# Mesoptier/ray-marching

Hardware: AMD Instinct MI355X
Metric: Mpixels/s at 1920x1080, 256-step march, 32-node SDF (higher is better)
Workload: dtype f32; 1 GPU; 1920x1080, g32 (31 commands / 111 words), 256 max steps, 16 rays/px, RGBA32F out; camera=still, kernel=0, specialized_kernel=True, jit_from_disk_cache=True, frames_in_flight=4

## Files before the change

ray-marching_amd/csrc/rm_abi.hip:

```cpp
#include <hip/hip_runtime.h>

#include <algorithm>
#include <cassert>
#include <cstdarg>
#include <cstdio>
#include <cstdlib>
#include <cmath>
#include <cstring>
#include <mutex>
#include <string>
#include <type_traits>
#include <vector>

#include "rm_abi.h"
#include "rm_abi_layout.h"
#include "rm_lds_layout.h"
#include "rm_decode.h"
#include "rm_jit.h"
#include "rm_device.h"
#include "rm_kernels.h"
#include "rm_interp.h"
#include "rm_kernel_v5.h"
#include "rm_query.h"
#include "rm_trace.h"
// ... 107 lines not shown
    DevBuf<char> d_swork, d_slayers, d_spoints, d_scontours, d_sattr;
    bool slice_valid = false;
    uint64_t slice_p = 0, slice_c = 0;
    uint32_t slice_layers = 0, slice_flags = 0;
    DevBuf<char> d_out;
    DevBuf<rm_uniforms> d_frames;
    int kernel = RM_KERNEL_DEFAULT;
    uint32_t refill_min_v5 = 0;
    bool cull = true;
    int balance = 3;
    int waves_per_tile = 0;
    bool wave_stats = false;
    DevBuf<unsigned long long> d_stats;
    size_t stats_valid_bytes = 0;
    DevBuf<uint32_t> d_cost, d_order;
    DevBuf<uint32_t> d_counters;
    DevBuf<uint32_t> d_measured;
    uint64_t measured_shape = 0;
    bool timing = false;
    double last_kernel_ms = 0.0;
    int specialize = 1;
    int out_format = RM_FORMAT_RGBA32F;
    int prune = 2;
    uint64_t prog_gen = 0;
    std::shared_ptr<rmjit::Entry> spec;
    uint64_t spec_gen = ~0ull;
    int spec_wpt = 0;
    int spec_pruned = 0;
    bool spec_stats = false;
    bool last_specialized = false;
// ... 198 lines not shown
    const RmDecoded& d = c->decoded;
    const V5Plan plan = plan_v5(c, L, lds);
    const bool units = plan.units;
    const int loop = plan.loop;
    c->last_loop = loop;
    const uint32_t n_tiles = ((L.W + 7u) / 8u) * ((L.rows + 7u) / 8u);
    hipFunction_t spec_fn = lds ? specialised_kernel(c, WPT) : nullptr;
    if (spec_fn) { L.spill_depth = 0u; L.n_tree = 0u; }
    if (L.n_mrec != 0u && !(spec_fn && c->spec && c->spec->material_walk))
        L.spill_depth = std::max(L.spill_depth, 2u * d.mat_spill_depth + 3u * d.mat_xform_depth);
    L.wave_dwords = rml::V5_WAVE_DWORDS - ((spec_fn && c->spec && c->spec->taps4 && L.n_mrec == 0u) ? rml::V5_TN_DWORDS : 0u);
    const size_t shmem = rml::MarchLds(WPT, L.wave_dwords, L.spill_depth, L.n_cone, L.n_slab, lds, L.n_rec, L.n_grp, L.n_tree, L.n_mrec != 0u).bytes;
    if (shmem > rml::kLdsLaunchLimit) return fail(c, RM_ERR_TOO_LARGE, "program needs %zu bytes of LDS per tile", shmem);
    if (int rc = c->d_cost.reserve(c, (size_t)n_tiles * n_frames)) return rc;
    if (int rc = c->d_order.reserve(c, (size_t)n_tiles * n_frames)) return rc;
    if (int rc = c->d_counters.reserve(c, (size_t)n_frames * 4u)) return rc;
    hipLaunchKernelGGL(rmk::rm_tile_pre_v5, dim3((n_tiles + rmk::V5_PRE_BLOCK - 1u) / rmk::V5_PRE_BLOCK, 1, n_frames),
                       dim3(64u * rmk::V5_PRE_TILES), rml::CullLds(L.n_cone, L.n_slab, true).bytes, s, L, c->d_cost.p, n_tiles);
    const uint32_t* prev = nullptr;
    uint32_t* measured = nullptr;
    if (c->balance == 3) {
        const size_t need = (size_t)n_tiles * n_frames;
        if (need > c->d_measured.cap) {
            if (int rc = c->d_measured.reserve(c, need)) return rc;
            c->measured_shape = 0;
        }
        const uint64_t shape = ((uint64_t)L.W << 40) ^ ((uint64_t)L.rows << 20) ^ ((uint64_t)L.strip_rows << 12) ^
                               ((uint64_t)L.strip_first << 6) ^ (uint64_t)L.strip_stride ^ ((uint64_t)n_frames << 52) ^ 1ull;
        if (c->measured_shape == shape) prev = c->d_measured.p;
        else HIP_TRY(c, hipMemsetAsync(c->d_measured.p, 0, need * sizeof(uint32_t), s));
        c->measured_shape = shape;
        measured = c->d_measured.p;
    }
    hipLaunchKernelGGL(rmk::rm_tile_sort_v5, dim3(n_frames), dim3(1024), 0, s, L, c->d_cost.p, c->d_order.p, c->d_counters.p,
                       n_tiles, (uint32_t)c->balance, prev);
    rmk::V5Work work{c->d_order.p, c->d_counters.p, measured};
    uint32_t per_cu = (uint32_t)std::min<size_t>(32u / WPT, (160u * 1024u) / shmem);
    if (per_cu < 1u) per_cu = 1u;
    if (per_cu > 24u / WPT) per_cu = 24u / WPT;
    const uint32_t n_wg = std::min<uint32_t>(n_tiles, (uint32_t)std::max(1, c->cu_count) * per_cu);
    dim3 grid(n_wg, 1, n_frames);
    if (int rc = ensure_stats(c, L, (size_t)n_wg * n_frames * WPT)) return rc;
    if (int rc = time_begin(c, s)) return rc;
    const bool ext = d.has_extensions || !d.is_tree;
    c->last_specialized = spec_fn != nullptr;
    const bool pruning = spec_fn ? (c->spec && c->spec_pruned != rmjit::PRUNE_NONE) : units && lds;
    const uint32_t refill_auto = c->refill_min_v5 != 0u ? c->refill_min_v5 : (pruning ? 64u : 1u);
    if (spec_fn) {
        uint32_t n_tiles_arg = n_tiles, refill = refill_auto;
        void* args[] = {&L, &work, &n_tiles_arg, &refill};
        hipError_t e = hipModuleLaunchKernel(spec_fn, grid.x, grid.y, grid.z, 64u * WPT, 1, 1, (unsigned)shmem, s, args, nullptr);
// ... 1994 lines not shown
```

ray-marching_amd/csrc/rm_kernel_v5.h:

```cpp
#pragma once
#include "rm_interp.h"
#include "rm_lds_layout.h"

namespace rmk {

typedef const __attribute__((address_space(3))) float* LdsF;
RM_DEV LdsF lds_vector_base(const void* generic_lds_ptr) {
    const uint32_t s = (uint32_t)(__SIZE_TYPE__)(const __attribute__((address_space(3))) void*)generic_lds_ptr;
    uint32_t v;
    asm("v_mov_b32 %0, %1" : "=v"(v) : "s"(s));
    return (LdsF)(__SIZE_TYPE__)v;
}
template <bool FAST>
RM_DEV float map_scene_spec(LdsF lp, float qx, float qy, float qz, unsigned long long need, unsigned long long live, SqrtGuard& tiny, uint32_t& n_eval);
#ifdef RM_JIT_MATERIAL_WALK
template <bool FAST>
RM_DEV uint32_t map_scene_material_spec(const RmRecord* __restrict__ mp, float qx, float qy, float qz, SqrtGuard& tiny);
#endif
#ifdef RM_JIT_TAPS4
template <bool FAST>
RM_DEV void map_scene_taps(LdsF lp, float cx, float cy, float cz, unsigned long long need, unsigned long long live, SqrtGuard& tiny, float (&f)[4]);
#endif

constexpr float kPruneAbs = 4.0e-6f;
// ... 330 lines not shown
        finite = finite && hx < inf && hy < inf && hz < inf;
        const float M = cull_margin(cx, cy, cz, hx + hy + hz, ro, min_dist, slack);
        slab[3u * slot] = make_float4((cx - hx - M) - ro.x, (cy - hy - M) - ro.y, (cz - hz - M) - ro.z, 0.0f);
        slab[3u * slot + 1u] = make_float4((cx + hx + M) - ro.x, (cy + hy + M) - ro.y, (cz + hz + M) - ro.z, 0.0f);
        const float Rk = __builtin_sqrtf((hx + M) * (hx + M) + (hy + M) * (hy + M) + (hz + M) * (hz + M)) * (1.0f + 1.0e-5f);
        const float mx = cx - ro.x, my = cy - ro.y, mz = cz - ro.z;
        const float mm = mx * mx + my * my + mz * mz;
        const float lim = mm * (1.0f - 4.0e-6f) - Rk * Rk * (1.0f + 4.0e-6f);
        float sv = -inf;
        if (lim > 0.0f && lim < inf) sv = __builtin_sqrtf(lim) * (1.0f - 1.0e-5f) - 1.0e-5f * __builtin_sqrtf(mm);
        slab[3u * slot + 2u] = make_float4(mx, my, mz, sv);
    }
    if (!finite || !(slack < inf)) atomicOr(veto, 1u);
}

RM_DEV bool ray_misses_scene_v5(const CullTables& T, float dx, float dy, float dz) {
    bool clear = *T.veto == 0u;
    unit_dir(dx, dy, dz);
    for (uint32_t k = 0; k < T.n_cone; k++) {
        const float4 a = T.cone[k];
        const float t = __builtin_fmaf(a.z, dz, __builtin_fmaf(a.y, dy, __builtin_fmaf(a.x, dx, -a.w)));
        clear = clear && (t < 0.0f);
        if ((k & 3u) == 3u && __ballot(clear) == 0ull) return false;
    }
    if (T.n_slab == 0u || __ballot(clear) == 0ull) return clear;
    const float tiny = 1.0e-30f;
    const float ix = __builtin_amdgcn_rcpf(__builtin_copysignf(fmax_(__builtin_fabsf(dx), tiny), dx));
    const float iy = __builtin_amdgcn_rcpf(__builtin_copysignf(fmax_(__builtin_fabsf(dy), tiny), dy));
    const float iz = __builtin_amdgcn_rcpf(__builtin_copysignf(fmax_(__builtin_fabsf(dz), tiny), dz));
    for (uint32_t k = 0; k < T.n_slab; k++) {
        const float4 c = T.slab[3u * k + 2u];
        const float t = __builtin_fmaf(c.z, dz, __builtin_fmaf(c.y, dy, __builtin_fmaf(c.x, dx, -c.w)));
        if (__ballot(clear && !(t < 0.0f)) == 0ull) continue;
        const float4 a = T.slab[3u * k], b = T.slab[3u * k + 1u];
        const float x1 = a.x * ix, x2 = b.x * ix, y1 = a.y * iy, y2 = b.y * iy, z1 = a.z * iz, z2 = b.z * iz;
        const float tn = fmax_(fmin_(x1, x2), fmax_(fmin_(y1, y2), fmin_(z1, z2)));
        const float tf = fmin_(fmax_(x1, x2), fmin_(fmax_(y1, y2), fmax_(z1, z2)));
        clear = clear && !(tf >= fmax_(tn, 0.0f));
        if (__ballot(clear) == 0ull) return false;
    }
    return clear;
}

template <bool CONE, class LoadRecord>
RM_DEV float ray_bound_v5(const LoadRecord& load, uint32_t n_rec, const V4& ro, float dx, float dy, float dz, float scale, float rho = 0.0f) {
    if (!CONE) unit_dir(dx, dy, dz);
    const float tiny = 1.0e-18f;
    const float ax = fmax_(__builtin_fabsf(dx), tiny), ay = fmax_(__builtin_fabsf(dy), tiny), az = fmax_(__builtin_fabsf(dz), tiny);
    const float ix = __builtin_amdgcn_rcpf(__builtin_copysignf(ax, dx)), iy = __builtin_amdgcn_rcpf(__builtin_copysignf(ay, dy));
    const float iz = __builtin_amdgcn_rcpf(__builtin_copysignf(az, dz));
    const float wxy = (ax * ay) * __builtin_amdgcn_rcpf(ax + ay), wxz = (ax * az) * __builtin_amdgcn_rcpf(ax + az);
    const float wyz = (ay * az) * __builtin_amdgcn_rcpf(ay + az);
    const float lower = 2.0e-6f * scale;
    const float inf = __uint_as_float(0x7F800000u);
    float acc = inf, spilled = inf;
// ... 63 lines not shown
    }
    return acc;
}
template <bool CONE, class LoadRecord>
RM_DEV bool ray_misses_by_bounds_v5(const LoadRecord& load, uint32_t n_rec, const V4& ro, float dx, float dy, float dz, float min_dist,
                                    float scale, float rho = 0.0f) {
    const float acc = ray_bound_v5<CONE>(load, n_rec, ro, dx, dy, dz, scale, rho);
    const float margin = fmax_(min_dist, 0.0f) * 1.01f + 1.0e-4f * scale;
    return acc > margin;
}

struct V5Work {
    const uint32_t* order;
    uint32_t* counters;
    uint32_t* measured;
};

RM_DEV float select_by_mask(float a, float b, unsigned long long m) {
    float r;
    asm("v_cndmask_b32_e64 %0, %1, %2, %3" : "=v"(r) : "v"(a), "v"(b), "s"(m));
    return r;
}
RM_DEV uint32_t select_by_mask(uint32_t a, uint32_t b, unsigned long long m) {
    uint32_t r;
    asm("v_cndmask_b32_e64 %0, %1, %2, %3" : "=v"(r) : "v"(a), "v"(b), "s"(m));
    return r;
}
RM_DEV bool lane_of(unsigned long long m, uint32_t lane) {
    uint32_t r;
    asm("v_cndmask_b32_e64 %0, 0, 1, %1" : "=v"(r) : "s"(m));
// ... 18 lines not shown
    float* sq_v = reinterpret_cast<float*>(wbase + WL::sq_v / 4u);
    uint32_t* hq_rid = wbase + WL::hq_rid / 4u;
    float* hq_v = reinterpret_cast<float*>(wbase + WL::hq_v / 4u);
    float* wxy = reinterpret_cast<float*>(wbase + WL::wxy / 4u);
    float* tn = reinterpret_cast<float*>(wbase + WL::tn / 4u);
    uint32_t* after = smem + V5_POOL + WPT * L.wave_dwords;
    float* spill = reinterpret_cast<float*>(after) + wave * (L.spill_depth * 64u) + lane;
    float4* t_cone = reinterpret_cast<float4*>(after + WPT * L.spill_depth * 64u);
    float4* t_slab = t_cone + L.n_cone;
    uint32_t* lprog = reinterpret_cast<uint32_t*>(t_slab + 3u * L.n_slab);
    uint32_t* s_next = lprog + (PROG_IN_LDS ? (L.n_rec + L.n_grp + L.n_tree) * 8u : 0u);
    uint32_t* s_tile = s_next + 1;
    uint32_t* s_veto = s_next + 2;
    float* s_off = reinterpret_cast<float*>(s_next + rml::kMarchCtlBytes / 4u);
    uint8_t* rmat = reinterpret_cast<uint8_t*>(s_next) + rml::kMarchCtlBytes + rml::kMarchOffBytes;
    const bool tagged = MAT && L.n_mrec != 0u;
    constexpr uint32_t TAP_IDLE = MAT ? 5u : 4u;
    const CullTables cullt{t_cone, t_slab, s_veto, L.n_cone, L.n_slab};

    rm_uniforms u = L.u;
    if (L.frames) u = L.frames[blockIdx.z];
    const uint32_t tiles_x = (L.W + 7u) / 8u;
    const uint32_t* order = work.order + (size_t)blockIdx.z * n_tiles;
    uint32_t* counters = work.counters + 4u * blockIdx.z;
    const uint32_t n_active = counters[0];

    const V4 ro = matvec(u.inv_view, 0.0f, 0.0f, 0.0f, 1.0f);
    const float prune_scale = L.scene_scale + ((__builtin_fabsf(ro.x) + __builtin_fabsf(ro.y)) + __builtin_fabsf(ro.z));
    const float eps = 0.0001f;
    if (PROG_IN_LDS) {
// ... 110 lines not shown
        s_next[3] = 0u;
    }
    __syncthreads();
    const uint32_t slot = *s_tile;
    if (slot >= n_active) break;
    const uint32_t tile = order[slot];
    const uint32_t tile_x = tile % tiles_x, tile_y = tile / tiles_x;
    n_tiles_done++;
    const unsigned long long tile_t0 = work.measured ? __builtin_amdgcn_s_memrealtime() : 0ull;

    if (lane < 16u) {
        const uint32_t k = lane & 7u, tx = tile_x * 8u + k, ty = tile_y * 8u + k;
        wxy[lane] = lane < 8u ? screen_x(tx < L.W ? tx : L.W - 1u, L.W)
                              : screen_y(rm_global_row(L, ty < L.rows ? ty : L.rows - 1u), L.H);
    }
    __builtin_amdgcn_fence(__ATOMIC_ACQ_REL, "wavefront");

    float dx = 0.f, dy = 0.f, dz = 0.f, sc = 0.f;
    constexpr uint32_t ITR_EMPTY = 0x80000000u, ITR_RETIRED = 0x40000000u;
    uint32_t itr = ITR_EMPTY;
    auto lane_empty = [&]() { return (int32_t)itr < 0; };
    auto lane_marching = [&]() { return itr < ITR_RETIRED; };
    const uint32_t iter_limit = L.max_iter << 10;
    float thr_base = inf_f;
    uint32_t rq_pos = 0u, rq_cnt = 0u, sq_n = 0u, hq_n = 0u;
    uint32_t tap_t = TAP_IDLE, tap_n = 0u;
    bool pool_open = true;

    auto flush_misses = [&]() {
        __builtin_amdgcn_fence(__ATOMIC_ACQ_REL, "wavefront");
// ... 16 lines not shown
                        }
                        uint32_t base = 0u;
                        if (lane == 0u) base = atomicAdd(s_next, 64u);
                        base = __builtin_amdgcn_readfirstlane(base);
                        if (base >= V5_POOL) { pool_open = false; continue; }
                        n_prod++;
                        const uint32_t blk = (uint32_t)(0xEDB87421A965FC30ull >> (4u * (base >> 6))) & 15u;
                        uint32_t ln = lane;
                        asm volatile("" : "+v"(ln));
                        const uint32_t bpx = 2u * (blk & 3u) + (ln & 1u), bpy = 2u * (blk >> 2) + ((ln >> 1) & 1u), s = ln >> 2;
                        const uint32_t r = s * 64u + bpy * 8u + bpx;
                        float gx, gy, gz;
                        gen_ray_at<true>(u.inv_proj, u.inv_view, ro, wxy[bpx], wxy[8u + bpy], s_off[2u * s], s_off[2u * s + 1u], gx, gy, gz);
                        const bool finite_d = __builtin_fabsf(gx) < inf_f && __builtin_fabsf(gy) < inf_f && __builtin_fabsf(gz) < inf_f;
                        const bool test_rays = (L.flags & 1u) != 0u && __builtin_amdgcn_readfirstlane(s_next[3]) < 4u;
                        bool culled = L.max_iter == 0u || (start == START_DONE && finite_d) || (test_rays && ray_misses_scene_v5(cullt, gx, gy, gz));
#if !defined(RM_JIT_TU) || defined(RM_JIT_BOUND_WALK)
                        if (test_rays && (L.flags & 32u) && (*s_veto & 1u) == 0u && bound_scale < 1.0e12f && __ballot(!culled) != 0ull)
                            culled = culled || ray_misses_by_bounds_v5<false>(load_record, L.n_rec, ro, gx, gy, gz, L.min_dist, bound_scale);
#endif
                        if (test_rays && base < 256u && __ballot(culled) == 0ull && lane == 0u) atomicAdd(&s_next[3], 1u);
                        if (culled) res[r] = miss_code(ro, gx, gy, gz);
                        const unsigned long long keep = __ballot(!culled);
                        if (!culled) {
                            const uint32_t e = lane_rank(keep);
                            rq_rid[e] = r;
                            rq_d[e] = gx; rq_d[V5_RQ + e] = gy; rq_d[2u * V5_RQ + e] = gz;
                        }
                        rq_pos = 0u;
                        rq_cnt = (uint32_t)__popcll(keep);
                        __builtin_amdgcn_fence(__ATOMIC_ACQ_REL, "wavefront");
// ... 269 lines not shown
    cone_out[0] = cx; cone_out[1] = cy; cone_out[2] = cz;
    cone_out[3] = cone_ok ? rho : __uint_as_float(0x7FC00000u);
    return cone_ok;
}
RM_DEV float cone_noise_v5(const rm_uniforms& u, const V4& ro, uint32_t W, uint32_t H) {
    const float bx = (1.0f + 16.0f / (float)W) + 0.75f / __builtin_fabsf(u.viewport_extent[0]);
    const float by = (1.0f + 16.0f / (float)H) + 0.75f / __builtin_fabsf(u.viewport_extent[1]);
    float mag = (__builtin_fabsf(ro.x) + __builtin_fabsf(ro.y)) + __builtin_fabsf(ro.z);
#pragma unroll
    for (int k = 0; k < 4; k++)
        mag += ((__builtin_fabsf(u.inv_view[4 * k]) + __builtin_fabsf(u.inv_view[1 + 4 * k])) + __builtin_fabsf(u.inv_view[2 + 4 * k])) *
               (((__builtin_fabsf(u.inv_proj[k]) * bx + __builtin_fabsf(u.inv_proj[k + 4]) * by) + __builtin_fabsf(u.inv_proj[k + 8])) +
                __builtin_fabsf(u.inv_proj[k + 12]));
    return 1.0e-6f * mag;
}
RM_DEV bool cone_misses_tables_v5(const CullTables& T, const float2* aux, const float (&cone)[4], bool cone_ok) {
    const float cx = cone[0], cy = cone[1], cz = cone[2], rho = cone[3];
    bool clear = cone_ok && *T.veto == 0u;
    for (uint32_t k = 0; k < T.n_cone; k++) {
        const float4 a = T.cone[k];
        const float t = __builtin_fmaf(aux[k].x, rho, __builtin_fmaf(a.z, cz, __builtin_fmaf(a.y, cy, a.x * cx)));
        clear = clear && (t < a.w);
        if ((k & 3u) == 3u && __ballot(clear) == 0ull) return false;
    }
    if (T.n_slab == 0u || __ballot(clear) == 0ull) return clear;
    const float tiny = 1.0e-30f;
    const float ix = __builtin_amdgcn_rcpf(__builtin_copysignf(fmax_(__builtin_fabsf(cx), tiny), cx));
    const float iy = __builtin_amdgcn_rcpf(__builtin_copysignf(fmax_(__builtin_fabsf(cy), tiny), cy));
    const float iz = __builtin_amdgcn_rcpf(__builtin_copysignf(fmax_(__builtin_fabsf(cz), tiny), cz));
    for (uint32_t k = 0; k < T.n_slab; k++) {
        const float4 c = T.slab[3u * k + 2u];
        const float2 x = aux[T.n_cone + k];
        const float t = __builtin_fmaf(x.x, rho, __builtin_fmaf(c.z, cz, __builtin_fmaf(c.y, cy, c.x * cx)));
        if (__ballot(clear && !(t < c.w)) == 0ull) continue;
        const float infl = x.y * rho;
        const float4 a = T.slab[3u * k], b = T.slab[3u * k + 1u];
        const float x1 = (a.x - infl) * ix, x2 = (b.x + infl) * ix, y1 = (a.y - infl) * iy, y2 = (b.y + infl) * iy;
        const float z1 = (a.z - infl) * iz, z2 = (b.z + infl) * iz;
        const float tn = fmax_(fmin_(x1, x2), fmax_(fmin_(y1, y2), fmin_(z1, z2)));
        const float tf = fmin_(fmax_(x1, x2), fmin_(fmax_(y1, y2), fmax_(z1, z2)));
        clear = clear && infl < __uint_as_float(0x7F800000u) && !(tf >= fmax_(tn, 0.0f));
        if (__ballot(clear) == 0ull) return false;
    }
    return clear;
}
RM_DEV bool pixel_misses_scene_v5(const CullTables& T, const float2* aux, const float* m_proj, const float* m_view, const float* off,
                                  const V4& ro, float sx, float sy, float noise, float (&cone_out)[4], float (&corner)[4][3]) {
    const float px[2] = {sx, sx}, py[2] = {sy, sy}, ox[2] = {off[0], off[24]}, oy[2] = {off[1], off[7]};
    const bool cone_ok = rect_cone_v5(m_proj, m_view, ro, px, py, ox, oy, noise, cone_out, corner);
    return cone_misses_tables_v5(T, aux, cone_out, cone_ok);
}

RM_DEV void pixel_aux_build_v5(const float4* t_cone, const float4* t_slab, uint32_t n_cone, uint32_t n_slab, float2* t_aux, uint32_t tid,
                               uint32_t n_threads) {
    const float up = 1.0f + 1.0e-6f;
    for (uint32_t k = tid; k < n_cone + n_slab; k += n_threads) {
        float4 m;
        float radius = 0.0f;
        if (k < n_cone) {
            m = t_cone[k];
        } else {
            const uint32_t j = k - n_cone;
            m = t_slab[3u * j + 2u];
            const float4 a = t_slab[3u * j], b = t_slab[3u * j + 1u];
            const float hx = b.x - a.x, hy = b.y - a.y, hz = b.z - a.z;
// ... 50 lines not shown
        gz_lo = fmin_(gz_lo, gz); gz_hi = fmax_(gz_hi, gz);
        uniform = uniform && gx == gx && gz == gz;
    }
    const float dx_lo = Cf * gx_hi, dx_hi = Cf * gx_lo, dz_lo = Cf * gz_hi, dz_hi = Cf * gz_lo;
    const float dev_x = fmax_(__builtin_fabsf(dx_lo), __builtin_fabsf(dx_hi)), dev_z = fmax_(__builtin_fabsf(dz_lo), __builtin_fabsf(dz_hi));
    const float del_x = 4.0f * (absC * inv_my) * (Ex + ((ax_hi + Ex) * inv_my) * Ey) + 2.0e-5f * ((1.0f + __builtin_fabsf(ro.x)) + dev_x);
    const float del_z = 4.0f * (absC * inv_my) * (Ez + ((az_hi + Ez) * inv_my) * Ey) + 2.0e-5f * ((1.0f + __builtin_fabsf(ro.z)) + dev_z);
    const float nx = __builtin_rintf(((ro.x + dx_lo) - del_x) + 0.5f), nz = __builtin_rintf(((ro.z + dz_lo) - del_z) + 0.5f);
    uniform = uniform && nx == __builtin_rintf(((ro.x + dx_hi) + del_x) + 0.5f) && nz == __builtin_rintf(((ro.z + dz_hi) + del_z) + 0.5f);
    code = (__float2int_rz(nx) ^ __float2int_rz(nz)) & 1;
    return uniform;
}

constexpr uint32_t V5_TILE_CLEAR = 1u, V5_TILE_SKY = 2u, V5_TILE_CELL = 4u, V5_TILE_CODE = 8u;
RM_DEV uint32_t tile_verdict_v5(const RmLaunch& L, const rm_uniforms& u, const V4& ro, const CullTables& T, const float2* aux, const float* off,
                                bool tables, bool all_miss, uint32_t tile_x, uint32_t tile_y, float (&cone)[4]) {
    const uint32_t row = rm_global_row(L, tile_y * 8u);
    const float px[2] = {screen_x(tile_x * 8u, L.W), screen_x(tile_x * 8u + 7u, L.W)};
    const float py[2] = {screen_y(row, L.H), screen_y(row + 7u, L.H)};
    const float ox[2] = {fmin_(off[0], off[24]), fmax_(off[0], off[24])}, oy[2] = {fmax_(off[1], off[7]), fmin_(off[1], off[7])};
    float corner[4][3];
    const bool cone_ok = rect_cone_v5(u.inv_proj, u.inv_view, ro, px, py, ox, oy, cone_noise_v5(u, ro, L.W, L.H), cone, corner);
    bool clear = cone_ok && all_miss;
    if (!all_miss && tables) clear = cone_misses_tables_v5(T, aux, cone, cone_ok);
    float bx = 0.0f, by = 0.0f;
#pragma unroll
    for (int a = 0; a < 2; a++) {
        bx = fmax_(bx, __builtin_fabsf(px[a] + ox[a]));
        by = fmax_(by, __builtin_fabsf(py[a] + oy[a]));
    }
    float mag;
    int code = 0;
    const bool sky = rect_sky_v5(u, ro, corner, bx, by, mag);
    const bool cell = !sky && rect_cell_v5(u, ro, corner, bx, by, mag, code);
    bool spread = false;
#pragma unroll
    for (uint32_t c = 1; c < 4u; c++) spread = spread || corner[c][0] != corner[0][0] || corner[c][1] != corner[0][1] || corner[c][2] != corner[0][2];
    if (!spread) return 0u;
    return (clear ? V5_TILE_CLEAR : 0u) | (sky ? V5_TILE_SKY : 0u) | (cell ? V5_TILE_CELL | (code ? V5_TILE_CODE : 0u) : 0u);
}

RM_DEV CullTables stage_cull_tables(const RmLaunch& L, const V4& ro, uint32_t* smem, const rm_uniforms* u, float* off, const float2** aux,
                                    uint32_t tid, uint32_t n_threads) {
    const rml::CullLds lds(L.n_cone, L.n_slab, aux != nullptr);
    uint32_t* s_veto = lds_at<uint32_t>(smem, lds.veto);
    float4* t_cone = lds_at<float4>(smem, lds.cone);
    float4* t_slab = lds_at<float4>(smem, lds.slab);
    const bool tables = (L.flags & 1u) != 0u;
    if (tid == 0u) *s_veto = 0u;
    if (off && tid < 16u) sample_offset(*u, tid >> 2, tid & 3u, off[2u * tid], off[2u * tid + 1u]);
    __syncthreads();
    if (tables)
        for (uint32_t k = tid; k < L.n_rec; k += n_threads) cull_build_v5(L.prog[k], ro, L.min_dist, L.smooth_slack, t_cone, t_slab, s_veto, L.bounds);
    __syncthreads();
    if (aux) {
        float2* t_aux = lds_at<float2>(smem, lds.aux);
        if (tables) pixel_aux_build_v5(t_cone, t_slab, L.n_cone, L.n_slab, t_aux, tid, n_threads);
        __syncthreads();
        *aux = t_aux;
    }
    return CullTables{t_cone, t_slab, s_veto, L.n_cone, L.n_slab};
}

__global__ __launch_bounds__(64 * V5_PRE_TILES) void rm_tile_pre_v5(RmLaunch L, uint32_t* cost, uint32_t n_tiles) {
    extern __shared__ __attribute__((aligned(16))) uint32_t smem[];
    const uint32_t tid = threadIdx.x, lane = tid & 63u, wave = tid >> 6;
    rm_uniforms u = L.u;
    if (L.frames) u = L.frames[blockIdx.z];
    const V4 ro = matvec(u.inv_view, 0.0f, 0.0f, 0.0f, 1.0f);
    const bool tables = (L.flags & 1u) != 0u;
    __shared__ float s_off[32];
    __shared__ float s_sxy[V5_PRE_TILES][128];
    __shared__ uint8_t s_code[V5_PRE_TILES][64 * 16];
    __shared__ uint8_t s_list[V5_PRE_TILES][64];
    __shared__ uint8_t s_verdict[V5_PRE_BLOCK];
    __shared__ uint32_t s_claim;
    if (tid == 0u) s_claim = 0u;
    const float2* t_aux;
    const CullTables cullt = stage_cull_tables(L, ro, smem, &u, s_off, &t_aux, tid, 64u * V5_PRE_TILES);
    const uint32_t* s_veto = cullt.veto;
    const uint32_t tiles_x = (L.W + 7u) / 8u;
    const float cone_noise = cone_noise_v5(u, ro, L.W, L.H);
  auto do_tile = [&](uint32_t tile) {
    const uint32_t tile_x = tile % tiles_x, tile_y = tile / tiles_x;
    const uint32_t tx = tile_x * 8u + (lane & 7u), ty = tile_y * 8u + (lane >> 3);
    const uint32_t px = tx < L.W ? tx : L.W - 1u, ry = ty < L.rows ? ty : L.rows - 1u;
    const float sx = screen_x(px, L.W), sy = screen_y(rm_global_row(L, ry), L.H);
    float mp[16], mv[16];
#pragma unroll
    for (int k = 0; k < 16; k++) {
        mp[k] = u.inv_proj[k]; mv[k] = u.inv_view[k];
        asm volatile("" : "+v"(mp[k]), "+v"(mv[k]));
    }
    bool clear;
    float corner[4][3];
    if (L.max_iter == 0u || !tables) {
        clear = L.max_iter == 0u;
#pragma unroll
        for (uint32_t c = 0; c < 4u; c++) {
            const uint32_t s = ((c & 1u) * 3u) * 4u + (c >> 1) * 3u;
            gen_ray_unnormalized_at(mp, mv, ro, sx, sy, s_off[2u * s], s_off[2u * s + 1u], corner[c][0], corner[c][1], corner[c][2]);
        }
    } else {
        float cone[4];
        clear = pixel_misses_scene_v5(cullt, t_aux, mp, mv, s_off, ro, sx, sy, cone_noise, cone, corner);
        const float bound_scale = bound_scale_prepass_v5(L, ro);
        if ((L.flags & 32u) && (*s_veto & 1u) == 0u && bound_scale < 1.0e12f && __ballot(!clear && cone[3] == cone[3]) != 0ull) {
            const ProgSmem prog{L.prog};
            auto load_record = [&](uint32_t i, uint32_t& op, float (&p)[7]) { prog.load(i, op, p); };
            const bool by_bounds = ray_misses_by_bounds_v5<true>(load_record, L.n_rec, ro, cone[0], cone[1], cone[2], L.min_dist, bound_scale, cone[3]);
            clear = clear || (cone[3] == cone[3] && by_bounds);
        }
    }
    const uint32_t pending = (uint32_t)__popcll(__ballot(!clear));
    if (lane == 0u) cost[(size_t)blockIdx.z * n_tiles + tile] = pending;
    if (pending != 0u) return;
    const float bx = __builtin_fabsf(sx) + __builtin_fabsf(s_off[0]), by = __builtin_fabsf(sy) + __builtin_fabsf(s_off[1]);
    float mag;
    const bool sky = rect_sky_v5(u, ro, corner, bx, by, mag);
    if (__ballot(!sky) == 0ull) {
// ... 48 lines not shown
            gen_ray_at<true>(mp, mv, ro, sx, sy, s_off[2u * s], s_off[2u * s + 1u], dx, dy, dz);
            const int c = shade_floor(ro.y, ro.x, ro.z, dx, dy, dz);
            float rg, b;
            gamma_of(c, rg, b);
            tr += rg;
            tg += rg;
            tb += b;
        }
    }
    if (tx < L.W && ty < L.rows) {
        store_pixel(L, blockIdx.z, (size_t)ty * L.W + tx, tr / 16.0f, tg / 16.0f, tb / 16.0f);
    }
  };
    const uint32_t first_tile = blockIdx.x * V5_PRE_BLOCK;
    if (tid < V5_PRE_BLOCK) {
        uint32_t v = 0u;
        if ((tables || L.max_iter == 0u) && L.strip_rows % 8u == 0u) {
            const uint32_t tile = first_tile + tid < n_tiles ? first_tile + tid : n_tiles - 1u;
            float cone[4];
            v = tile_verdict_v5(L, u, ro, cullt, t_aux, s_off, tables, L.max_iter == 0u, tile % tiles_x, tile / tiles_x, cone);
            if (!(v & V5_TILE_CLEAR) || !(v & (V5_TILE_SKY | V5_TILE_CELL))) v = 0u;
        }
        s_verdict[tid] = (uint8_t)v;
    }
    __syncthreads();
    for (;;) {
        uint32_t t = 0u;
        if (lane == 0u) t = atomicAdd(&s_claim, 1u);
        t = (uint32_t)__builtin_amdgcn_readfirstlane((int)t);
        if (t >= V5_PRE_BLOCK || first_tile + t >= n_tiles) break;
        const uint32_t tile = first_tile + t, v = s_verdict[t];
        if (v == 0u) {
            do_tile(tile);
            __builtin_amdgcn_fence(__ATOMIC_ACQ_REL, "wavefront");
            continue;
        }
        float tr = 0.0f, tb = 0.0f;
        if (v & V5_TILE_CELL) {
            const float g = 0.2f * (float)((v & V5_TILE_CODE) ? 1 : 0);
            const float rg = __builtin_sqrtf(0.1f + g), b = __builtin_sqrtf(0.2f + g);
            for (uint32_t s = 0; s < 16u; s++) {
                tr += rg;
                tb += b;
            }
        }
        const uint32_t tx = (tile % tiles_x) * 8u + (lane & 7u), ty = (tile / tiles_x) * 8u + (lane >> 3);
        if (lane == 0u) cost[(size_t)blockIdx.z * n_tiles + tile] = 0u;
        if (tx < L.W && ty < L.rows) store_pixel(L, blockIdx.z, (size_t)ty * L.W + tx, tr / 16.0f, tr / 16.0f, tb / 16.0f);
// ... 89 lines not shown
        }
    }
}
#endif

#if !defined(RM_JIT_TU)
__global__ __launch_bounds__(64) void rm_selftest_cull_rays_kernel(RmLaunch L, V4 ro, const float* dirs, uint32_t n, uint32_t* out_flags,
                                                                   float* out_bound) {
    extern __shared__ __attribute__((aligned(16))) uint32_t smem[];
    const uint32_t tid = threadIdx.x;
    const bool tables = (L.flags & 1u) != 0u;
    const CullTables cullt = stage_cull_tables(L, ro, smem, nullptr, nullptr, nullptr, tid, 64u);
    const uint32_t i = blockIdx.x * 64u + tid, j = i < n ? i : n - 1u;
    const float gx = dirs[3u * j], gy = dirs[3u * j + 1u], gz = dirs[3u * j + 2u];
    const uint32_t veto = *cullt.veto;
    const bool clear = tables && ray_misses_scene_v5(cullt, gx, gy, gz);
    const float bound_scale = bound_scale_march_v5(L, ro);
    const bool walk = tables && (L.flags & 32u) && (veto & 1u) == 0u && bound_scale < 1.0e12f;
    float acc = __uint_as_float(0x7FC00000u);
    bool by_bounds = false;
    if (walk) {
        const ProgSmem prog{L.prog};
        auto load_record = [&](uint32_t r, uint32_t& op, float (&p)[7]) { prog.load(r, op, p); };
        acc = ray_bound_v5<false>(load_record, L.n_rec, ro, gx, gy, gz, bound_scale);
        by_bounds = ray_misses_by_bounds_v5<false>(load_record, L.n_rec, ro, gx, gy, gz, L.min_dist, bound_scale);
    }
    if (i < n) {
        out_flags[i] = (clear ? 1u : 0u) | ((tables && veto == 0u) ? 2u : 0u) | (walk ? 4u : 0u) | (by_bounds ? 8u : 0u) | (veto << 8);
        out_bound[i] = acc;
    }
}
// ... 4 lines not shown
    const rm_uniforms u = L.u;
    const V4 ro = matvec(u.inv_view, 0.0f, 0.0f, 0.0f, 1.0f);
    const bool tables = (L.flags & 1u) != 0u;
    const float2* t_aux;
    const CullTables cullt = stage_cull_tables(L, ro, smem, &u, s_off, &t_aux, tid, 64u);
    const uint32_t i = blockIdx.x * 64u + tid, j = i < n ? i : n - 1u;
    const float sx = screen_x(xy[2u * j], L.W), sy = screen_y(rm_global_row(L, xy[2u * j + 1u]), L.H);
    float mp[16], mv[16];
#pragma unroll
    for (int k = 0; k < 16; k++) { mp[k] = u.inv_proj[k]; mv[k] = u.inv_view[k]; }
    const float nan = __uint_as_float(0x7FC00000u), cone_noise = cone_noise_v5(u, ro, L.W, L.H);
    float cone[4] = {nan, nan, nan, nan}, corner[4][3], acc = nan;
    bool clear = false, walk = false, by_bounds = false;
    const uint32_t veto = *cullt.veto;
    if (tables) {
        clear = pixel_misses_scene_v5(cullt, t_aux, mp, mv, s_off, ro, sx, sy, cone_noise, cone, corner);
        const float bound_scale = bound_scale_prepass_v5(L, ro);
        walk = (L.flags & 32u) && (veto & 1u) == 0u && bound_scale < 1.0e12f && cone[3] == cone[3];
        if (__ballot(walk) != 0ull) {
            const ProgSmem prog{L.prog};
            auto load_record = [&](uint32_t r, uint32_t& op, float (&p)[7]) { prog.load(r, op, p); };
            const float b = ray_bound_v5<true>(load_record, L.n_rec, ro, cone[0], cone[1], cone[2], bound_scale, cone[3]);
            const bool v = ray_misses_by_bounds_v5<true>(load_record, L.n_rec, ro, cone[0], cone[1], cone[2], L.min_dist, bound_scale, cone[3]);
            if (walk) { acc = b; by_bounds = v; }
        }
    }
    if (i < n) {
        float* o = out + 8u * (size_t)i;
        o[0] = cone[0]; o[1] = cone[1]; o[2] = cone[2]; o[3] = cone[3]; o[4] = acc;
        o[5] = __uint_as_float((clear ? 1u : 0u) | ((tables && veto == 0u) ? 2u : 0u) | (walk ? 4u : 0u) | (by_bounds ? 8u : 0u));
        o[6] = 0.0f; o[7] = 0.0f;
    }
}
__global__ __launch_bounds__(64) void rm_selftest_cull_tiles_kernel(RmLaunch L, const uint32_t* xy, uint32_t n, float* out) {
    extern __shared__ __attribute__((aligned(16))) uint32_t smem[];
    __shared__ float s_off[32];
    const uint32_t tid = threadIdx.x;
    const rm_uniforms u = L.u;
    const V4 ro = matvec(u.inv_view, 0.0f, 0.0f, 0.0f, 1.0f);
    const bool tables = (L.flags & 1u) != 0u;
    const float2* t_aux;
    const CullTables cullt = stage_cull_tables(L, ro, smem, &u, s_off, &t_aux, tid, 64u);
    const uint32_t i = blockIdx.x * 64u + tid, j = i < n ? i : n - 1u;
    float cone[4];
    const uint32_t v = tile_verdict_v5(L, u, ro, cullt, t_aux, s_off, tables, L.max_iter == 0u, xy[2u * j], xy[2u * j + 1u], cone);
    if (i < n) {
        float* o = out + 8u * (size_t)i;
        o[0] = cone[0]; o[1] = cone[1]; o[2] = cone[2]; o[3] = cone[3];
        o[4] = (v & V5_TILE_CODE) ? 1.0f : 0.0f;
        o[5] = __uint_as_float(((v & V5_TILE_CLEAR) ? 1u : 0u) | ((v & V5_TILE_SKY) ? 2u : 0u) | ((v & V5_TILE_CELL) ? 4u : 0u) |
                               ((tables && *cullt.veto == 0u) ? 8u : 0u));
        o[6] = 0.0f; o[7] = 0.0f;
    }
}
__global__ __launch_bounds__(64) void rm_selftest_cull_waves_kernel(RmLaunch L, V4 ro, const float* pos, const float* thr, const unsigned long long* live,
                                                                    float extra_margin, unsigned long long* out) {
    extern __shared__ __attribute__((aligned(16))) uint32_t smem[];
    const uint32_t lane = threadIdx.x, w = blockIdx.x;
    stage_units(smem, L.prog + L.n_rec, L.n_grp, lane, 64u);
    __syncthreads();
    const float x = pos[(3u * w) * 64u + lane], y = pos[(3u * w + 1u) * 64u + lane], z = pos[(3u * w + 2u) * 64u + lane];
    const unsigned long long live_mask = live[w];
    const bool is_live = ((live_mask >> lane) & 1ull) != 0ull;
    const float prune_scale = prune_scale_v5(L, ro);
    unsigned long long need;
    if (L.unit_mode == RM_UNITS_LATTICE) need = wave_cull_lattice(smem, L.n_grp, x, y, z, thr[64u * w + lane], is_live, live_mask);
    else need = wave_cull_blend(smem, L.n_grp, L.unit_kmax, x, y, z, extra_margin, prune_scale, is_live, live_mask);
// ... 6 lines not shown
```

Before: 6706 Mpixels/s.

## Record per-tile cull-table touch masks and test only touched entries per ray

The tile prepass now computes, for each 8x8 tile cone, a bitmask of the cone and slab cull entries it cannot rule out, and stores it in a new per-tile buffer. The per-pixel prepass and the march kernel's per-ray cull test then iterate only over the set bits instead of every cone and slab entry. This removes redundant cull-table tests for rays whose tile cone already clears most entries, at the cost of an extra buffer write and read, one LDS slot, and slightly more divergent mask-iteration loops. Scenes with more than 32 entries fall back to the full test.

```diff
diff --git a/ray-marching_amd/csrc/rm_abi.hip b/ray-marching_amd/csrc/rm_abi.hip
--- a/ray-marching_amd/csrc/rm_abi.hip
+++ b/ray-marching_amd/csrc/rm_abi.hip
@@ -145,6 +145,7 @@
     DevBuf<unsigned long long> d_stats;
     size_t stats_valid_bytes = 0;
     DevBuf<uint32_t> d_cost, d_order;
+    DevBuf<uint32_t> d_masks;
     DevBuf<uint32_t> d_counters;
     DevBuf<uint32_t> d_measured;
     uint64_t measured_shape = 0;
@@ -373,9 +374,10 @@
     if (shmem > rml::kLdsLaunchLimit) return fail(c, RM_ERR_TOO_LARGE, "program needs %zu bytes of LDS per tile", shmem);
     if (int rc = c->d_cost.reserve(c, (size_t)n_tiles * n_frames)) return rc;
     if (int rc = c->d_order.reserve(c, (size_t)n_tiles * n_frames)) return rc;
+    if (int rc = c->d_masks.reserve(c, (size_t)n_tiles * n_frames)) return rc;
     if (int rc = c->d_counters.reserve(c, (size_t)n_frames * 4u)) return rc;
     hipLaunchKernelGGL(rmk::rm_tile_pre_v5, dim3((n_tiles + rmk::V5_PRE_BLOCK - 1u) / rmk::V5_PRE_BLOCK, 1, n_frames),
-                       dim3(64u * rmk::V5_PRE_TILES), rml::CullLds(L.n_cone, L.n_slab, true).bytes, s, L, c->d_cost.p, n_tiles);
+                       dim3(64u * rmk::V5_PRE_TILES), rml::CullLds(L.n_cone, L.n_slab, true).bytes, s, L, c->d_cost.p, c->d_masks.p, n_tiles);
     const uint32_t* prev = nullptr;
     uint32_t* measured = nullptr;
     if (c->balance == 3) {
@@ -393,7 +395,7 @@
     }
     hipLaunchKernelGGL(rmk::rm_tile_sort_v5, dim3(n_frames), dim3(1024), 0, s, L, c->d_cost.p, c->d_order.p, c->d_counters.p,
                        n_tiles, (uint32_t)c->balance, prev);
-    rmk::V5Work work{c->d_order.p, c->d_counters.p, measured};
+    rmk::V5Work work{c->d_order.p, c->d_counters.p, measured, c->d_masks.p};
     uint32_t per_cu = (uint32_t)std::min<size_t>(32u / WPT, (160u * 1024u) / shmem);
     if (per_cu < 1u) per_cu = 1u;
     if (per_cu > 24u / WPT) per_cu = 24u / WPT;
diff --git a/ray-marching_amd/csrc/rm_kernel_v5.h b/ray-marching_amd/csrc/rm_kernel_v5.h
--- a/ray-marching_amd/csrc/rm_kernel_v5.h
+++ b/ray-marching_amd/csrc/rm_kernel_v5.h
@@ -368,31 +368,48 @@
     if (!finite || !(slack < inf)) atomicOr(veto, 1u);
 }
 
-RM_DEV bool ray_misses_scene_v5(const CullTables& T, float dx, float dy, float dz) {
+constexpr uint32_t V5_MASK_ALL = 0xFFFFFFFFu;
+RM_DEV uint32_t mask_cone_bits(uint32_t mask, uint32_t n_cone) { return n_cone >= 32u ? mask : mask & ((1u << n_cone) - 1u); }
+RM_DEV uint32_t mask_slab_bits(uint32_t mask, uint32_t n_cone) { return n_cone >= 32u ? 0u : mask >> n_cone; }
+
+RM_DEV void ray_cone_entry_v5(const CullTables& T, uint32_t k, float dx, float dy, float dz, bool& clear) {
+    const float4 a = T.cone[k];
+    const float t = __builtin_fmaf(a.z, dz, __builtin_fmaf(a.y, dy, __builtin_fmaf(a.x, dx, -a.w)));
+    clear = clear && (t < 0.0f);
+}
+RM_DEV bool ray_slab_entry_v5(const CullTables& T, uint32_t k, float dx, float dy, float dz, float ix, float iy, float iz, bool& clear) {
+    const float4 c = T.slab[3u * k + 2u];
+    const float t = __builtin_fmaf(c.z, dz, __builtin_fmaf(c.y, dy, __builtin_fmaf(c.x, dx, -c.w)));
+    if (__ballot(clear && !(t < 0.0f)) == 0ull) return false;
+    const float4 a = T.slab[3u * k], b = T.slab[3u * k + 1u];
+    const float x1 = a.x * ix, x2 = b.x * ix, y1 = a.y * iy, y2 = b.y * iy, z1 = a.z * iz, z2 = b.z * iz;
+    const float tn = fmax_(fmin_(x1, x2), fmax_(fmin_(y1, y2), fmin_(z1, z2)));
+    const float tf = fmin_(fmax_(x1, x2), fmin_(fmax_(y1, y2), fmax_(z1, z2)));
+    clear = clear && !(tf >= fmax_(tn, 0.0f));
+    return __ballot(clear) == 0ull;
+}
+RM_DEV float slab_rcp_v5(float d) { return __builtin_amdgcn_rcpf(__builtin_copysignf(fmax_(__builtin_fabsf(d), 1.0e-30f), d)); }
+
+RM_DEV bool ray_misses_scene_v5(const CullTables& T, uint32_t mask, float dx, float dy, float dz) {
     bool clear = *T.veto == 0u;
     unit_dir(dx, dy, dz);
+    if (mask != V5_MASK_ALL) {
+        for (uint32_t m = mask_cone_bits(mask, T.n_cone); m != 0u; m &= m - 1u) ray_cone_entry_v5(T, (uint32_t)__builtin_ctz(m), dx, dy, dz, clear);
+        const uint32_t ms = mask_slab_bits(mask, T.n_cone);
+        if (ms == 0u || __ballot(clear) == 0ull) return clear;
+        const float ix = slab_rcp_v5(dx), iy = slab_rcp_v5(dy), iz = slab_rcp_v5(dz);
+        for (uint32_t m = ms; m != 0u; m &= m - 1u)
+            if (ray_slab_entry_v5(T, (uint32_t)__builtin_ctz(m), dx, dy, dz, ix, iy, iz, clear)) return false;
+        return clear;
+    }
     for (uint32_t k = 0; k < T.n_cone; k++) {
-        const float4 a = T.cone[k];
-        const float t = __builtin_fmaf(a.z, dz, __builtin_fmaf(a.y, dy, __builtin_fmaf(a.x, dx, -a.w)));
-        clear = clear && (t < 0.0f);
+        ray_cone_entry_v5(T, k, dx, dy, dz, clear);
         if ((k & 3u) == 3u && __ballot(clear) == 0ull) return false;
     }
     if (T.n_slab == 0u || __ballot(clear) == 0ull) return clear;
-    const float tiny = 1.0e-30f;
-    const float ix = __builtin_amdgcn_rcpf(__builtin_copysignf(fmax_(__builtin_fabsf(dx), tiny), dx));
-    const float iy = __builtin_amdgcn_rcpf(__builtin_copysignf(fmax_(__builtin_fabsf(dy), tiny), dy));
-    const float iz = __builtin_amdgcn_rcpf(__builtin_copysignf(fmax_(__builtin_fabsf(dz), tiny), dz));
-    for (uint32_t k = 0; k < T.n_slab; k++) {
-        const float4 c = T.slab[3u * k + 2u];
-        const float t = __builtin_fmaf(c.z, dz, __builtin_fmaf(c.y, dy, __builtin_fmaf(c.x, dx, -c.w)));
-        if (__ballot(clear && !(t < 0.0f)) == 0ull) continue;
-        const float4 a = T.slab[3u * k], b = T.slab[3u * k + 1u];
-        const float x1 = a.x * ix, x2 = b.x * ix, y1 = a.y * iy, y2 = b.y * iy, z1 = a.z * iz, z2 = b.z * iz;
-        const float tn = fmax_(fmin_(x1, x2), fmax_(fmin_(y1, y2), fmin_(z1, z2)));
-        const float tf = fmin_(fmax_(x1, x2), fmin_(fmax_(y1, y2), fmax_(z1, z2)));
-        clear = clear && !(tf >= fmax_(tn, 0.0f));
-        if (__ballot(clear) == 0ull) return false;
-    }
+    const float ix = slab_rcp_v5(dx), iy = slab_rcp_v5(dy), iz = slab_rcp_v5(dz);
+    for (uint32_t k = 0; k < T.n_slab; k++)
+        if (ray_slab_entry_v5(T, k, dx, dy, dz, ix, iy, iz, clear)) return false;
     return clear;
 }
 
@@ -486,6 +503,7 @@
     const uint32_t* order;
     uint32_t* counters;
     uint32_t* measured;
+    const uint32_t* masks;
 };
 
 RM_DEV float select_by_mask(float a, float b, unsigned long long m) {
@@ -534,6 +552,7 @@
     uint32_t* s_veto = s_next + 2;
     float* s_off = reinterpret_cast<float*>(s_next + rml::kMarchCtlBytes / 4u);
     uint8_t* rmat = reinterpret_cast<uint8_t*>(s_next) + rml::kMarchCtlBytes + rml::kMarchOffBytes;
+    uint32_t* s_mask = reinterpret_cast<uint32_t*>(rmat + (MAT && L.n_mrec != 0u ? V5_POOL : 0u));
     const bool tagged = MAT && L.n_mrec != 0u;
     constexpr uint32_t TAP_IDLE = MAT ? 5u : 4u;
     const CullTables cullt{t_cone, t_slab, s_veto, L.n_cone, L.n_slab};
@@ -674,6 +693,7 @@
         wxy[lane] = lane < 8u ? screen_x(tx < L.W ? tx : L.W - 1u, L.W)
                               : screen_y(rm_global_row(L, ty < L.rows ? ty : L.rows - 1u), L.H);
     }
+    if (lane == 0u) *s_mask = work.masks[(size_t)blockIdx.z * n_tiles + tile];
     __builtin_amdgcn_fence(__ATOMIC_ACQ_REL, "wavefront");
 
     float dx = 0.f, dy = 0.f, dz = 0.f, sc = 0.f;
@@ -720,7 +740,7 @@
                         gen_ray_at<true>(u.inv_proj, u.inv_view, ro, wxy[bpx], wxy[8u + bpy], s_off[2u * s], s_off[2u * s + 1u], gx, gy, gz);
                         const bool finite_d = __builtin_fabsf(gx) < inf_f && __builtin_fabsf(gy) < inf_f && __builtin_fabsf(gz) < inf_f;
                         const bool test_rays = (L.flags & 1u) != 0u && __builtin_amdgcn_readfirstlane(s_next[3]) < 4u;
-                        bool culled = L.max_iter == 0u || (start == START_DONE && finite_d) || (test_rays && ray_misses_scene_v5(cullt, gx, gy, gz));
+                        bool culled = L.max_iter == 0u || (start == START_DONE && finite_d) || (test_rays && ray_misses_scene_v5(cullt, __builtin_amdgcn_readfirstlane(*s_mask), gx, gy, gz));
 #if !defined(RM_JIT_TU) || defined(RM_JIT_BOUND_WALK)
                         if (test_rays && (L.flags & 32u) && (*s_veto & 1u) == 0u && bound_scale < 1.0e12f && __ballot(!culled) != 0ull)
                             culled = culled || ray_misses_by_bounds_v5<false>(load_record, L.n_rec, ro, gx, gy, gz, L.min_dist, bound_scale);
@@ -1020,41 +1040,85 @@
                 __builtin_fabsf(u.inv_proj[k + 12]));
     return 1.0e-6f * mag;
 }
-RM_DEV bool cone_misses_tables_v5(const CullTables& T, const float2* aux, const float (&cone)[4], bool cone_ok) {
+RM_DEV bool cone_clears_cone_entry_v5(const CullTables& T, const float2* aux, uint32_t k, float cx, float cy, float cz, float rho) {
+    const float4 a = T.cone[k];
+    const float t = __builtin_fmaf(aux[k].x, rho, __builtin_fmaf(a.z, cz, __builtin_fmaf(a.y, cy, a.x * cx)));
+    return t < a.w;
+}
+RM_DEV bool cone_clears_slab_sphere_v5(const CullTables& T, const float2* aux, uint32_t k, float cx, float cy, float cz, float rho) {
+    const float4 c = T.slab[3u * k + 2u];
+    const float t = __builtin_fmaf(aux[T.n_cone + k].x, rho, __builtin_fmaf(c.z, cz, __builtin_fmaf(c.y, cy, c.x * cx)));
+    return t < c.w;
+}
+RM_DEV bool cone_clears_slab_box_v5(const CullTables& T, const float2* aux, uint32_t k, float rho, float ix, float iy, float iz) {
+    const float infl = aux[T.n_cone + k].y * rho;
+    const float4 a = T.slab[3u * k], b = T.slab[3u * k + 1u];
+    const float x1 = (a.x - infl) * ix, x2 = (b.x + infl) * ix, y1 = (a.y - infl) * iy, y2 = (b.y + infl) * iy;
+    const float z1 = (a.z - infl) * iz, z2 = (b.z + infl) * iz;
+    const float tn = fmax_(fmin_(x1, x2), fmax_(fmin_(y1, y2), fmin_(z1, z2)));
+    const float tf = fmin_(fmax_(x1, x2), fmin_(fmax_(y1, y2), fmax_(z1, z2)));
+    return infl < __uint_as_float(0x7F800000u) && !(tf >= fmax_(tn, 0.0f));
+}
+RM_DEV bool cone_misses_tables_v5(const CullTables& T, const float2* aux, const float (&cone)[4], bool cone_ok, uint32_t mask) {
     const float cx = cone[0], cy = cone[1], cz = cone[2], rho = cone[3];
     bool clear = cone_ok && *T.veto == 0u;
+    if (mask != V5_MASK_ALL) {
+        for (uint32_t m = mask_cone_bits(mask, T.n_cone); m != 0u; m &= m - 1u)
+            clear = clear && cone_clears_cone_entry_v5(T, aux, (uint32_t)__builtin_ctz(m), cx, cy, cz, rho);
+        const uint32_t ms = mask_slab_bits(mask, T.n_cone);
+        if (ms == 0u || __ballot(clear) == 0ull) return clear;
+        const float ix = slab_rcp_v5(cx), iy = slab_rcp_v5(cy), iz = slab_rcp_v5(cz);
+        for (uint32_t m = ms; m != 0u; m &= m - 1u) {
+            const uint32_t k = (uint32_t)__builtin_ctz(m);
+            if (__ballot(clear && !cone_clears_slab_sphere_v5(T, aux, k, cx, cy, cz, rho)) == 0ull) continue;
+            clear = clear && cone_clears_slab_box_v5(T, aux, k, rho, ix, iy, iz);
+            if (__ballot(clear) == 0ull) return false;
+        }
+        return clear;
+    }
     for (uint32_t k = 0; k < T.n_cone; k++) {
-        const float4 a = T.cone[k];
-        const float t = __builtin_fmaf(aux[k].x, rho, __builtin_fmaf(a.z, cz, __builtin_fmaf(a.y, cy, a.x * cx)));
-        clear = clear && (t < a.w);
+        clear = clear && cone_clears_cone_entry_v5(T, aux, k, cx, cy, cz, rho);
         if ((k & 3u) == 3u && __ballot(clear) == 0ull) return false;
     }
     if (T.n_slab == 0u || __ballot(clear) == 0ull) return clear;
-    const float tiny = 1.0e-30f;
-    const float ix = __builtin_amdgcn_rcpf(__builtin_copysignf(fmax_(__builtin_fabsf(cx), tiny), cx));
-    const float iy = __builtin_amdgcn_rcpf(__builtin_copysignf(fmax_(__builtin_fabsf(cy), tiny), cy));
-    const float iz = __builtin_amdgcn_rcpf(__builtin_copysignf(fmax_(__builtin_fabsf(cz), tiny), cz));
+    const float ix = slab_rcp_v5(cx), iy = slab_rcp_v5(cy), iz = slab_rcp_v5(cz);
     for (uint32_t k = 0; k < T.n_slab; k++) {
-        const float4 c = T.slab[3u * k + 2u];
-        const float2 x = aux[T.n_cone + k];
-        const float t = __builtin_fmaf(x.x, rho, __builtin_fmaf(c.z, cz, __builtin_fmaf(c.y, cy, c.x * cx)));
-        if (__ballot(clear && !(t < c.w)) == 0ull) continue;
-        const float infl = x.y * rho;
-        const float4 a = T.slab[3u * k], b = T.slab[3u * k + 1u];
-        const float x1 = (a.x - infl) * ix, x2 = (b.x + infl) * ix, y1 = (a.y - infl) * iy, y2 = (b.y + infl) * iy;
-        const float z1 = (a.z - infl) * iz, z2 = (b.z + infl) * iz;
-        const float tn = fmax_(fmin_(x1, x2), fmax_(fmin_(y1, y2), fmin_(z1, z2)));
-        const float tf = fmin_(fmax_(x1, x2), fmin_(fmax_(y1, y2), fmax_(z1, z2)));
-        clear = clear && infl < __uint_as_float(0x7F800000u) && !(tf >= fmax_(tn, 0.0f));
+        if (__ballot(clear && !cone_clears_slab_sphere_v5(T, aux, k, cx, cy, cz, rho)) == 0ull) continue;
+        clear = clear && cone_clears_slab_box_v5(T, aux, k, rho, ix, iy, iz);
         if (__ballot(clear) == 0ull) return false;
     }
     return clear;
 }
+RM_DEV bool tile_touch_mask_v5(const CullTables& T, const float2* aux, const float (&cone)[4], bool cone_ok, uint32_t& mask) {
+    const float cx = cone[0], cy = cone[1], cz = cone[2], rho = cone[3];
+    bool clear = cone_ok && *T.veto == 0u;
+    uint32_t touched = 0u;
+    for (uint32_t k = 0; k < T.n_cone; k++) {
+        const bool ok = cone_clears_cone_entry_v5(T, aux, k, cx, cy, cz, rho);
+        clear = clear && ok;
+        touched |= ok ? 0u : 1u << k;
+    }
+    if (T.n_slab != 0u) {
+        const float ix = slab_rcp_v5(cx), iy = slab_rcp_v5(cy), iz = slab_rcp_v5(cz);
+        for (uint32_t k = 0; k < T.n_slab; k++) {
+            const bool sphere_ok = cone_clears_slab_sphere_v5(T, aux, k, cx, cy, cz, rho);
+            if (__ballot(!sphere_ok) == 0ull) continue;
+            const bool wave_ran_box = __ballot(clear && !sphere_ok) != 0ull;
+            const bool box_decides = clear && wave_ran_box;
+            const bool box_ok = cone_clears_slab_box_v5(T, aux, k, rho, ix, iy, iz);
+            const bool ok = box_decides ? box_ok : (sphere_ok || box_ok);
+            clear = clear && ok;
+            touched |= ok ? 0u : 1u << (T.n_cone + k);
+        }
+    }
+    mask = touched;
+    return clear;
+}
 RM_DEV bool pixel_misses_scene_v5(const CullTables& T, const float2* aux, const float* m_proj, const float* m_view, const float* off,
-                                  const V4& ro, float sx, float sy, float noise, float (&cone_out)[4], float (&corner)[4][3]) {
+                                  const V4& ro, float sx, float sy, float noise, uint32_t mask, float (&cone_out)[4], float (&corner)[4][3]) {
     const float px[2] = {sx, sx}, py[2] = {sy, sy}, ox[2] = {off[0], off[24]}, oy[2] = {off[1], off[7]};
     const bool cone_ok = rect_cone_v5(m_proj, m_view, ro, px, py, ox, oy, noise, cone_out, corner);
-    return cone_misses_tables_v5(T, aux, cone_out, cone_ok);
+    return cone_misses_tables_v5(T, aux, cone_out, cone_ok, mask);
 }
 
 RM_DEV void pixel_aux_build_v5(const float4* t_cone, const float4* t_slab, uint32_t n_cone, uint32_t n_slab, float2* t_aux, uint32_t tid,
@@ -1135,7 +1199,7 @@
 
 constexpr uint32_t V5_TILE_CLEAR = 1u, V5_TILE_SKY = 2u, V5_TILE_CELL = 4u, V5_TILE_CODE = 8u;
 RM_DEV uint32_t tile_verdict_v5(const RmLaunch& L, const rm_uniforms& u, const V4& ro, const CullTables& T, const float2* aux, const float* off,
-                                bool tables, bool all_miss, uint32_t tile_x, uint32_t tile_y, float (&cone)[4]) {
+                                bool tables, bool all_miss, uint32_t tile_x, uint32_t tile_y, float (&cone)[4], uint32_t& mask) {
     const uint32_t row = rm_global_row(L, tile_y * 8u);
     const float px[2] = {screen_x(tile_x * 8u, L.W), screen_x(tile_x * 8u + 7u, L.W)};
     const float py[2] = {screen_y(row, L.H), screen_y(row + 7u, L.H)};
@@ -1143,7 +1207,16 @@
     float corner[4][3];
     const bool cone_ok = rect_cone_v5(u.inv_proj, u.inv_view, ro, px, py, ox, oy, cone_noise_v5(u, ro, L.W, L.H), cone, corner);
     bool clear = cone_ok && all_miss;
-    if (!all_miss && tables) clear = cone_misses_tables_v5(T, aux, cone, cone_ok);
+    mask = V5_MASK_ALL;
+    if (!all_miss && tables) {
+        if (T.n_cone + T.n_slab <= 32u) {
+            uint32_t touched;
+            clear = tile_touch_mask_v5(T, aux, cone, cone_ok, touched);
+            if (cone_ok && *T.veto == 0u) mask = touched;
+        } else {
+            clear = cone_misses_tables_v5(T, aux, cone, cone_ok, V5_MASK_ALL);
+        }
+    }
     float bx = 0.0f, by = 0.0f;
 #pragma unroll
     for (int a = 0; a < 2; a++) {
@@ -1157,7 +1230,10 @@
     bool spread = false;
 #pragma unroll
     for (uint32_t c = 1; c < 4u; c++) spread = spread || corner[c][0] != corner[0][0] || corner[c][1] != corner[0][1] || corner[c][2] != corner[0][2];
-    if (!spread) return 0u;
+    if (!spread) {
+        mask = V5_MASK_ALL;
+        return 0u;
+    }
     return (clear ? V5_TILE_CLEAR : 0u) | (sky ? V5_TILE_SKY : 0u) | (cell ? V5_TILE_CELL | (code ? V5_TILE_CODE : 0u) : 0u);
 }
 
@@ -1183,7 +1259,7 @@
     return CullTables{t_cone, t_slab, s_veto, L.n_cone, L.n_slab};
 }
 
-__global__ __launch_bounds__(64 * V5_PRE_TILES) void rm_tile_pre_v5(RmLaunch L, uint32_t* cost, uint32_t n_tiles) {
+__global__ __launch_bounds__(64 * V5_PRE_TILES) void rm_tile_pre_v5(RmLaunch L, uint32_t* cost, uint32_t* masks, uint32_t n_tiles) {
     extern __shared__ __attribute__((aligned(16))) uint32_t smem[];
     const uint32_t tid = threadIdx.x, lane = tid & 63u, wave = tid >> 6;
     rm_uniforms u = L.u;
@@ -1195,6 +1271,7 @@
     __shared__ uint8_t s_code[V5_PRE_TILES][64 * 16];
     __shared__ uint8_t s_list[V5_PRE_TILES][64];
     __shared__ uint8_t s_verdict[V5_PRE_BLOCK];
+    __shared__ uint32_t s_mask[V5_PRE_BLOCK];
     __shared__ uint32_t s_claim;
     if (tid == 0u) s_claim = 0u;
     const float2* t_aux;
@@ -1202,7 +1279,7 @@
     const uint32_t* s_veto = cullt.veto;
     const uint32_t tiles_x = (L.W + 7u) / 8u;
     const float cone_noise = cone_noise_v5(u, ro, L.W, L.H);
-  auto do_tile = [&](uint32_t tile) {
+  auto do_tile = [&](uint32_t tile, uint32_t tile_mask) {
     const uint32_t tile_x = tile % tiles_x, tile_y = tile / tiles_x;
     const uint32_t tx = tile_x * 8u + (lane & 7u), ty = tile_y * 8u + (lane >> 3);
     const uint32_t px = tx < L.W ? tx : L.W - 1u, ry = ty < L.rows ? ty : L.rows - 1u;
@@ -1224,7 +1301,7 @@
         }
     } else {
         float cone[4];
-        clear = pixel_misses_scene_v5(cullt, t_aux, mp, mv, s_off, ro, sx, sy, cone_noise, cone, corner);
+        clear = pixel_misses_scene_v5(cullt, t_aux, mp, mv, s_off, ro, sx, sy, cone_noise, tile_mask, cone, corner);
         const float bound_scale = bound_scale_prepass_v5(L, ro);
         if ((L.flags & 32u) && (*s_veto & 1u) == 0u && bound_scale < 1.0e12f && __ballot(!clear && cone[3] == cone[3]) != 0ull) {
             const ProgSmem prog{L.prog};
@@ -1303,14 +1380,16 @@
   };
     const uint32_t first_tile = blockIdx.x * V5_PRE_BLOCK;
     if (tid < V5_PRE_BLOCK) {
-        uint32_t v = 0u;
+        uint32_t v = 0u, mask = V5_MASK_ALL;
         if ((tables || L.max_iter == 0u) && L.strip_rows % 8u == 0u) {
             const uint32_t tile = first_tile + tid < n_tiles ? first_tile + tid : n_tiles - 1u;
             float cone[4];
-            v = tile_verdict_v5(L, u, ro, cullt, t_aux, s_off, tables, L.max_iter == 0u, tile % tiles_x, tile / tiles_x, cone);
+            v = tile_verdict_v5(L, u, ro, cullt, t_aux, s_off, tables, L.max_iter == 0u, tile % tiles_x, tile / tiles_x, cone, mask);
             if (!(v & V5_TILE_CLEAR) || !(v & (V5_TILE_SKY | V5_TILE_CELL))) v = 0u;
         }
         s_verdict[tid] = (uint8_t)v;
+        s_mask[tid] = mask;
+        if (first_tile + tid < n_tiles) masks[(size_t)blockIdx.z * n_tiles + first_tile + tid] = mask;
     }
     __syncthreads();
     for (;;) {
@@ -1320,7 +1399,7 @@
         if (t >= V5_PRE_BLOCK || first_tile + t >= n_tiles) break;
         const uint32_t tile = first_tile + t, v = s_verdict[t];
         if (v == 0u) {
-            do_tile(tile);
+            do_tile(tile, (uint32_t)__builtin_amdgcn_readfirstlane((int)s_mask[t]));
             __builtin_amdgcn_fence(__ATOMIC_ACQ_REL, "wavefront");
             continue;
         }
@@ -1440,7 +1519,7 @@
     const uint32_t i = blockIdx.x * 64u + tid, j = i < n ? i : n - 1u;
     const float gx = dirs[3u * j], gy = dirs[3u * j + 1u], gz = dirs[3u * j + 2u];
     const uint32_t veto = *cullt.veto;
-    const bool clear = tables && ray_misses_scene_v5(cullt, gx, gy, gz);
+    const bool clear = tables && ray_misses_scene_v5(cullt, V5_MASK_ALL, gx, gy, gz);
     const float bound_scale = bound_scale_march_v5(L, ro);
     const bool walk = tables && (L.flags & 32u) && (veto & 1u) == 0u && bound_scale < 1.0e12f;
     float acc = __uint_as_float(0x7FC00000u);
@@ -1475,7 +1554,7 @@
     bool clear = false, walk = false, by_bounds = false;
     const uint32_t veto = *cullt.veto;
     if (tables) {
-        clear = pixel_misses_scene_v5(cullt, t_aux, mp, mv, s_off, ro, sx, sy, cone_noise, cone, corner);
+        clear = pixel_misses_scene_v5(cullt, t_aux, mp, mv, s_off, ro, sx, sy, cone_noise, V5_MASK_ALL, cone, corner);
         const float bound_scale = bound_scale_prepass_v5(L, ro);
         walk = (L.flags & 32u) && (veto & 1u) == 0u && bound_scale < 1.0e12f && cone[3] == cone[3];
         if (__ballot(walk) != 0ull) {
@@ -1504,14 +1583,16 @@
     const CullTables cullt = stage_cull_tables(L, ro, smem, &u, s_off, &t_aux, tid, 64u);
     const uint32_t i = blockIdx.x * 64u + tid, j = i < n ? i : n - 1u;
     float cone[4];
-    const uint32_t v = tile_verdict_v5(L, u, ro, cullt, t_aux, s_off, tables, L.max_iter == 0u, xy[2u * j], xy[2u * j + 1u], cone);
+    uint32_t mask;
+    const uint32_t v = tile_verdict_v5(L, u, ro, cullt, t_aux, s_off, tables, L.max_iter == 0u, xy[2u * j], xy[2u * j + 1u], cone, mask);
+    if (L.strip_rows % 8u != 0u) mask = V5_MASK_ALL;
     if (i < n) {
         float* o = out + 8u * (size_t)i;
         o[0] = cone[0]; o[1] = cone[1]; o[2] = cone[2]; o[3] = cone[3];
         o[4] = (v & V5_TILE_CODE) ? 1.0f : 0.0f;
         o[5] = __uint_as_float(((v & V5_TILE_CLEAR) ? 1u : 0u) | ((v & V5_TILE_SKY) ? 2u : 0u) | ((v & V5_TILE_CELL) ? 4u : 0u) |
                                ((tables && *cullt.veto == 0u) ? 8u : 0u));
-        o[6] = 0.0f; o[7] = 0.0f;
+        o[6] = __uint_as_float(mask); o[7] = __uint_as_float(L.n_cone + L.n_slab);
     }
 }
 __global__ __launch_bounds__(64) void rm_selftest_cull_waves_kernel(RmLaunch L, V4 ro, const float* pos, const float* thr, const unsigned long long* live,
```

New measurement: 6870 Mpixels/s, median of 6. +2.4%, better.
